# vitasoftAI/ImageRetrievalResearch

Hardware: AMD Instinct MI355X
Metric: images/sec embed + queries/sec top-k@100k-gallery, EffNet-B3a 224^2 (higher is better)
Workload: dtype bf16

## Files before the change

imageretrievalresearch_amd/csrc/gemm_bf16.hip:

```cpp
#include "ops.h"
#include "../../include/mi355_retrieval.h"

#include <stdlib.h>

namespace mi355 {

typedef __bf16 bf16x8 __attribute__((ext_vector_type(8)));
typedef float f32x4 __attribute__((ext_vector_type(4)));
typedef unsigned u32x4 __attribute__((ext_vector_type(4)));
typedef unsigned u32x2 __attribute__((ext_vector_type(2)));

__device__ __forceinline__ float lo_bf(unsigned u) { return __uint_as_float(u << 16); }
__device__ __forceinline__ float hi_bf(unsigned u) { return __uint_as_float(u & 0xffff0000u); }

__device__ __forceinline__ u32x4 gate_chunk(u32x4 v, const float* __restrict__ gp, int relu6) {
    const f32x4 g0 = *reinterpret_cast<const f32x4*>(gp);
    const f32x4 g1 = *reinterpret_cast<const f32x4*>(gp + 4);
    float f[8] = {lo_bf(v.x) * g0.x, hi_bf(v.x) * g0.y, lo_bf(v.y) * g0.z, hi_bf(v.y) * g0.w,
                  lo_bf(v.z) * g1.x, hi_bf(v.z) * g1.y, lo_bf(v.w) * g1.z, hi_bf(v.w) * g1.w};
    if (relu6) {
#pragma unroll
        for (int i = 0; i < 8; ++i) f[i] = fminf(fmaxf(f[i], 0.f), 6.f);
    }
    u32x4 o;
    o.x = pack2bf(f[0], f[1]); o.y = pack2bf(f[2], f[3]); o.z = pack2bf(f[4], f[5]); o.w = pack2bf(f[6], f[7]);
    return o;
}

__device__ __forceinline__ u32x4 gate_chunk_regs(u32x4 v, f32x4 g0, f32x4 g1, int relu6) {
    float f[8] = {lo_bf(v.x) * g0.x, hi_bf(v.x) * g0.y, lo_bf(v.y) * g0.z, hi_bf(v.y) * g0.w,
                  lo_bf(v.z) * g1.x, hi_bf(v.z) * g1.y, lo_bf(v.w) * g1.z, hi_bf(v.w) * g1.w};
    if (relu6) {
#pragma unroll
        for (int i = 0; i < 8; ++i) f[i] = fminf(fmaxf(f[i], 0.f), 6.f);
    }
    u32x4 o;
    o.x = pack2bf(f[0], f[1]); o.y = pack2bf(f[2], f[3]); o.z = pack2bf(f[4], f[5]); o.w = pack2bf(f[6], f[7]);
    return o;
}

__device__ __forceinline__ u32x4 relu6_chunk(u32x4 v) {
    float f[8] = {lo_bf(v.x), hi_bf(v.x), lo_bf(v.y), hi_bf(v.y), lo_bf(v.z), hi_bf(v.z), lo_bf(v.w), hi_bf(v.w)};
#pragma unroll
    for (int i = 0; i < 8; ++i) f[i] = fminf(fmaxf(f[i], 0.f), 6.f);
    u32x4 o;
    o.x = pack2bf(f[0], f[1]); o.y = pack2bf(f[2], f[3]); o.z = pack2bf(f[4], f[5]); o.w = pack2bf(f[6], f[7]);
    return o;
}

template <int WM, int NT, int BK>
__global__ __launch_bounds__(256) void k_gemm_bf16(const GemmArgs g, const int n_tiles, const int nwg) {
    constexpr int BM = 64 * WM;
    constexpr int BN = NT * 16;
    constexpr int LD = BK + 8;
    constexpr int KC = BK / 8;
    constexpr int A_ITERS = BM * KC / 256;
    constexpr int W_ITERS = (BN * KC + 255) / 256;
    constexpr int CLD = BN + 8;
    extern __shared__ __attribute__((aligned(16))) bf16_t smem[];
    bf16_t* As = smem;
    bf16_t* Ws = smem + 2 * BM * LD;

    const int tid = threadIdx.x;
    const int lane = tid & 63;
    const int wave = tid >> 6;

    int logical;
    {
        const int bid = blockIdx.x;
        const int q = nwg >> 3, r = nwg & 7, xcd = bid & 7;
        logical = (xcd < r ? xcd * (q + 1) : r * (q + 1) + (xcd - r) * q) + (bid >> 3);
    }
    const int mb = logical / n_tiles, nb = logical - mb * n_tiles;
    const int m0 = mb * BM;
    const int n0 = nb * BN;
    const int Npad = (g.N + 15) & ~15;

    const bf16_t* a_ptr[A_ITERS];
    const float* a_gate[A_ITERS];
    bool a_ok[A_ITERS];
    int a_lds[A_ITERS], a_k[A_ITERS];
#pragma unroll
    for (int i = 0; i < A_ITERS; ++i) {
        const int id = tid + 256 * i;
        const int row = id / KC, c = id % KC;
        const int m = m0 + row;
        a_ok[i] = m < g.M;
        a_k[i] = c * 8;
        a_lds[i] = row * LD + c * 8;
        a_ptr[i] = g.A + (size_t)(a_ok[i] ? m : 0) * g.lda + c * 8;
        a_gate[i] = g.gate ? g.gate + (size_t)((a_ok[i] ? m : 0) / g.rows_per_img) * g.gate_ld + c * 8 : nullptr;
    }

    u32x4 ra[A_ITERS], rw[W_ITERS];
    auto load_tile = [&](int k0) {
#pragma unroll
        for (int i = 0; i < A_ITERS; ++i) {
            u32x4 v = {0u, 0u, 0u, 0u};
            if (a_ok[i] && (k0 + a_k[i]) < g.K) {
                v = *reinterpret_cast<const u32x4*>(a_ptr[i] + k0);
                if (g.gate) v = gate_chunk(v, a_gate[i] + k0, g.a_relu6);
                else if (g.a_relu6) v = relu6_chunk(v);
            }
            ra[i] = v;
        }
#pragma unroll
        for (int i = 0; i < W_ITERS; ++i) {
            const int id = tid + 256 * i;
            const int row = id / KC, c = id % KC;
            u32x4 v = {0u, 0u, 0u, 0u};
            if (row < BN && (n0 + row) < Npad && (k0 + c * 8) < g.ldw)
                v = *reinterpret_cast<const u32x4*>(g.W + (size_t)(n0 + row) * g.ldw + k0 + c * 8);
            rw[i] = v;
        }
    };
    auto store_tile = [&](int buf) {
#pragma unroll
        for (int i = 0; i < A_ITERS; ++i) *reinterpret_cast<u32x4*>(&As[buf * BM * LD + a_lds[i]]) = ra[i];
#pragma unroll
        for (int i = 0; i < W_ITERS; ++i) {
            const int id = tid + 256 * i;
            const int row = id / KC, c = id % KC;
            if (row < BN) *reinterpret_cast<u32x4*>(&Ws[buf * BN * LD + row * LD + c * 8]) = rw[i];
        }
    };

    f32x4 acc[NT][WM];
#pragma unroll
    for (int i = 0; i < NT; ++i)
#pragma unroll
        for (int j = 0; j < WM; ++j) acc[i][j] = (f32x4){0.f, 0.f, 0.f, 0.f};

    const int nt = (g.K + BK - 1) / BK;
    load_tile(0);
    store_tile(0);
    __syncthreads();

    const int fr = lane & 15;
    const int fk = (lane >> 4) * 8;
    for (int t = 0; t < nt; ++t) {
        const int buf = t & 1;
        if (t + 1 < nt) load_tile((t + 1) * BK);
        const bf16_t* as = As + buf * BM * LD;
        const bf16_t* ws = Ws + buf * BN * LD;
#pragma unroll
        for (int ks = 0; ks < BK / 32; ++ks) {
            bf16x8 af[WM];
#pragma unroll
            for (int mi = 0; mi < WM; ++mi)
                af[mi] = *reinterpret_cast<const bf16x8*>(&as[(wave * 16 * WM + mi * 16 + fr) * LD + ks * 32 + fk]);
            constexpr int WG = NT % 4 == 0 ? 4 : (NT % 3 == 0 ? 3 : 2);
#pragma unroll
            for (int n0i = 0; n0i < NT; n0i += WG) {
                bf16x8 wf[WG];
#pragma unroll
                for (int q = 0; q < WG; ++q)
                    wf[q] = *reinterpret_cast<const bf16x8*>(&ws[((n0i + q) * 16 + fr) * LD + ks * 32 + fk]);
                __builtin_amdgcn_sched_barrier(0);
#pragma unroll
                for (int q = 0; q < WG; ++q)
#pragma unroll
                    for (int mi = 0; mi < WM; ++mi)
                        acc[n0i + q][mi] = __builtin_amdgcn_mfma_f32_16x16x32_bf16(wf[q], af[mi], acc[n0i + q][mi], 0, 0, 0);
            }
        }
        if (t + 1 < nt) store_tile(buf ^ 1);
        __syncthreads();
    }

    MI355_ACT_DISPATCH(g.act, {
_Pragma("unroll")
        for (int ni = 0; ni < NT; ++ni) {
            const int n = n0 + ni * 16 + (lane >> 4) * 4;
            f32x4 b = {0.f, 0.f, 0.f, 0.f};
            if (n < Npad) b = *reinterpret_cast<const f32x4*>(g.bias + n);
_Pragma("unroll")
            for (int mi = 0; mi < WM; ++mi) {
                acc[ni][mi].x = act_c<ACT>(acc[ni][mi].x + b.x); acc[ni][mi].y = act_c<ACT>(acc[ni][mi].y + b.y);
                acc[ni][mi].z = act_c<ACT>(acc[ni][mi].z + b.z); acc[ni][mi].w = act_c<ACT>(acc[ni][mi].w + b.w);
            }
        }
    })
    const bool staged = (!g.out_f32) && (g.res == nullptr);
    if (staged) {
        bf16_t* Cs = smem;
#pragma unroll
        for (int mi = 0; mi < WM; ++mi) {
            const int ml = wave * 16 * WM + mi * 16 + fr;
#pragma unroll
            for (int ni = 0; ni < NT; ++ni) {
                const int nl = ni * 16 + (lane >> 4) * 4;
                u32x2 o;
                o.x = pack2bf(acc[ni][mi].x, acc[ni][mi].y);
                o.y = pack2bf(acc[ni][mi].z, acc[ni][mi].w);
                *reinterpret_cast<u32x2*>(&Cs[ml * CLD + nl]) = o;
            }
        }
        __syncthreads();
        constexpr int CPR = BN / 8;
        for (int id = tid; id < BM * CPR; id += 256) {
            const int row = id / CPR, c = id - row * CPR;
            const int m = m0 + row, n = n0 + c * 8;
            if (m < g.M && n < g.N)
                *reinterpret_cast<u32x4*>((bf16_t*)g.out + (size_t)m * g.ldo + n) =
                    *reinterpret_cast<const u32x4*>(&Cs[row * CLD + c * 8]);
        }
        return;
    }
#pragma unroll
    for (int mi = 0; mi < WM; ++mi) {
        const int m = m0 + wave * 16 * WM + mi * 16 + fr;
        if (m >= g.M) continue;
#pragma unroll
        for (int ni = 0; ni < NT; ++ni) {
            const int n = n0 + ni * 16 + (lane >> 4) * 4;
            if (n >= g.N) continue;
            float v[4] = {acc[ni][mi].x, acc[ni][mi].y, acc[ni][mi].z, acc[ni][mi].w};
            const bool res_vec = g.res && (n + 3 < g.res_n);
            const bool res_part = g.res && !res_vec && (n < g.res_n);
            if (n + 3 < g.N && !res_part) {
                if (res_vec) {
                    const u32x2 rr = *reinterpret_cast<const u32x2*>(g.res + (size_t)m * g.ldr + n);
                    v[0] += lo_bf(rr.x); v[1] += hi_bf(rr.x); v[2] += lo_bf(rr.y); v[3] += hi_bf(rr.y);
                }
                if (g.out_f32) {
                    float* o = (float*)g.out + (size_t)m * g.ldo + n;
                    o[0] = v[0]; o[1] = v[1]; o[2] = v[2]; o[3] = v[3];
                } else {
                    u32x2 o;
                    o.x = pack2bf(v[0], v[1]);
                    o.y = pack2bf(v[2], v[3]);
                    *reinterpret_cast<u32x2*>((bf16_t*)g.out + (size_t)m * g.ldo + n) = o;
                }
            } else {
#pragma unroll
                for (int r = 0; r < 4; ++r) {
                    if (n + r < g.N) {
                        float x = v[r];
                        if (g.res && n + r < g.res_n) x += bf2f(g.res[(size_t)m * g.ldr + n + r]);
                        if (g.out_f32) ((float*)g.out)[(size_t)m * g.ldo + n + r] = x;
                        else ((bf16_t*)g.out)[(size_t)m * g.ldo + n + r] = f2bf(x);
                    }
                }
            }
        }
    }
}

constexpr int BG_BM = 128, BG_BN = 128, BG_BK = 64;

__device__ __forceinline__ void glds16(const bf16_t* gsrc, bf16_t* lds_dst) {
    __builtin_amdgcn_global_load_lds((const __attribute__((address_space(1))) void*)gsrc,
                                     (__attribute__((address_space(3))) void*)lds_dst, 16, 0, 0);
}

template <bool GATED, bool KTAIL, int BKT = 64>
__global__ __launch_bounds__(256, BKT == 32 ? 3 : 1) void k_gemm_big(const GemmArgs g, const int n_tiles, const int nwg) {
    constexpr int MI = GATED ? 2 : 4;
    constexpr int NI = GATED ? 8 : 4;
    static_assert(BKT == 64 || (BKT == 32 && !GATED), "stage depths");
    constexpr int PPW = BKT / 16;
    constexpr int RPP = 512 / BKT;
    constexpr int CPRW = BKT / 8;
    extern __shared__ __attribute__((aligned(16))) bf16_t bsm[];
    bf16_t* As = bsm;
    bf16_t* Ws = bsm + 2 * BG_BM * BKT;
    auto swz = [](int row) { return BKT == 64 ? ((row >> 1) & 7) : ((0 - (row >> 2)) & 3); };
    const int tid = threadIdx.x, lane = tid & 63, wave = tid >> 6;
    int logical;
    {
        const int bid = blockIdx.x;
        const int q = nwg >> 3, r = nwg & 7, xcd = bid & 7;
        logical = (xcd < r ? xcd * (q + 1) : r * (q + 1) + (xcd - r) * q) + (bid >> 3);
    }
    const int mb = logical / n_tiles, nb = logical - mb * n_tiles;
    const int m0 = mb * BG_BM, n0 = nb * BG_BN;
    const int Npad = (g.N + 15) & ~15;

    const bf16_t* a_src[PPW];
    const bf16_t* w_src[PPW];
    int k_off[PPW];
    bool a_ok[PPW], w_ok[PPW];
#pragma unroll
    for (int i = 0; i < PPW; ++i) {
        const int row = (wave * PPW + i) * RPP + lane / CPRW;
        const int lchunk = (lane % CPRW) ^ swz(row);
        k_off[i] = lchunk * 8;
        a_ok[i] = (m0 + row) < g.M;
        w_ok[i] = (n0 + row) < Npad;
        a_src[i] = g.A + (size_t)(a_ok[i] ? m0 + row : 0) * g.lda + lchunk * 8;
        w_src[i] = g.W + (size_t)(w_ok[i] ? n0 + row : 0) * g.ldw + lchunk * 8;
    }
    auto stage = [&](int buf, int k0) {
#pragma unroll
        for (int i = 0; i < PPW; ++i) {
            const int piece = wave * PPW + i;
            const bf16_t* pa = KTAIL ? ((a_ok[i] && k0 + k_off[i] < g.K) ? a_src[i] + k0 : g.zeros) : a_src[i] + k0;
            const bf16_t* pw = KTAIL ? ((w_ok[i] && k0 + k_off[i] < g.ldw) ? w_src[i] + k0 : g.zeros) : w_src[i] + k0;
            glds16(pa, As + buf * BG_BM * BKT + piece * 512);
            glds16(pw, Ws + buf * BG_BN * BKT + piece * 512);
        }
    };

    const int wm = GATED ? wave : (wave >> 1), wn = GATED ? 0 : (wave & 1);
    const int fr = lane & 15, fq = lane >> 4;
    const int row_base = wm * (MI * 16), col_base = wn * (NI * 16);
// ... 43 lines not shown
        const bf16_t* as = As + buf * BG_BM * BKT;
        const bf16_t* ws = Ws + buf * BG_BN * BKT;
#pragma unroll
        for (int ks = 0; ks < BKT / 32; ++ks) {
            bf16x8 af[MI], wf[NI];
#pragma unroll
            for (int i = 0; i < MI; ++i) {
                const int ra = row_base + i * 16 + fr;
                u32x4 v = *reinterpret_cast<const u32x4*>(&as[ra * BKT + (((ks * 4 + fq) ^ swz(ra)) << 3)]);
                if (GATED) {
                    if (g.gate) v = gate_chunk_regs(v, gcur[i][ks][0], gcur[i][ks][1], g.a_relu6);
                    else if (g.a_relu6) v = relu6_chunk(v);
                }
                af[i] = *reinterpret_cast<bf16x8*>(&v);
            }
#pragma unroll
            for (int i = 0; i < NI; ++i) {
                const int rw = col_base + i * 16 + fr;
                wf[i] = *reinterpret_cast<const bf16x8*>(&ws[rw * BKT + (((ks * 4 + fq) ^ swz(rw)) << 3)]);
            }
#pragma unroll
            for (int ni = 0; ni < NI; ++ni)
#pragma unroll
                for (int mi = 0; mi < MI; ++mi)
                    acc[ni][mi] = __builtin_amdgcn_mfma_f32_16x16x32_bf16(wf[ni], af[mi], acc[ni][mi], 0, 0, 0);
        }
        __syncthreads();
    }

    if (!GATED && g.ln_stats) {
        float mean[MI], rstd[MI];
#pragma unroll
        for (int mi = 0; mi < MI; ++mi) {
            const int m = min(m0 + row_base + mi * 16 + fr, g.M - 1);
            const mi355_f32x2 st = *reinterpret_cast<const mi355_f32x2*>(g.ln_stats + (size_t)m * 2);
            mean[mi] = st.x; rstd[mi] = st.y;
        }
#pragma unroll
        for (int ni = 0; ni < NI; ++ni) {
            const int n = n0 + col_base + ni * 16 + fq * 4;
            f32x4 cs = {0.f, 0.f, 0.f, 0.f};
            if (n < Npad) cs = *reinterpret_cast<const f32x4*>(g.ln_colsum + n);
#pragma unroll
            for (int mi = 0; mi < MI; ++mi) {
                acc[ni][mi].x = rstd[mi] * (acc[ni][mi].x - mean[mi] * cs.x); acc[ni][mi].y = rstd[mi] * (acc[ni][mi].y - mean[mi] * cs.y);
                acc[ni][mi].z = rstd[mi] * (acc[ni][mi].z - mean[mi] * cs.z); acc[ni][mi].w = rstd[mi] * (acc[ni][mi].w - mean[mi] * cs.w);
            }
        }
    }
    MI355_ACT_DISPATCH(g.act, {
_Pragma("unroll")
        for (int ni = 0; ni < NI; ++ni) {
            const int n = n0 + col_base + ni * 16 + fq * 4;
            f32x4 b = {0.f, 0.f, 0.f, 0.f};
            if (n < Npad) b = *reinterpret_cast<const f32x4*>(g.bias + n);
_Pragma("unroll")
            for (int mi = 0; mi < MI; ++mi) {
                acc[ni][mi].x = act_c<ACT>(acc[ni][mi].x + b.x); acc[ni][mi].y = act_c<ACT>(acc[ni][mi].y + b.y);
                acc[ni][mi].z = act_c<ACT>(acc[ni][mi].z + b.z); acc[ni][mi].w = act_c<ACT>(acc[ni][mi].w + b.w);
            }
        }
    })
    const bool staged = (!g.out_f32) && (g.res == nullptr);
    if (staged) {
        constexpr int CLD = BG_BN + 8;
        bf16_t* Cs = bsm;
#pragma unroll
        for (int mi = 0; mi < MI; ++mi) {
            const int ml = row_base + mi * 16 + fr;
#pragma unroll
            for (int ni = 0; ni < NI; ++ni) {
                const int nl = col_base + ni * 16 + fq * 4;
                u32x2 o;
                o.x = pack2bf(acc[ni][mi].x, acc[ni][mi].y);
                o.y = pack2bf(acc[ni][mi].z, acc[ni][mi].w);
                *reinterpret_cast<u32x2*>(&Cs[ml * CLD + nl]) = o;
            }
        }
        __syncthreads();
        constexpr int CPR = BG_BN / 8;
        for (int id = tid; id < BG_BM * CPR; id += 256) {
            const int row = id / CPR, c = id - row * CPR;
            const int m = m0 + row, n = n0 + c * 8;
            if (m < g.M && n < g.N)
                *reinterpret_cast<u32x4*>((bf16_t*)g.out + (size_t)m * g.ldo + n) =
                    *reinterpret_cast<const u32x4*>(&Cs[row * CLD + c * 8]);
        }
        return;
    }
    if (!g.out_f32 && g.res_n >= g.N) {
        constexpr int FLD = BG_BN + 4;
        float* Cf = reinterpret_cast<float*>(bsm);
        constexpr int HALVES = BKT == 32 ? 2 : 1, HROWS = BG_BM / HALVES;
#pragma unroll
        for (int h = 0; h < HALVES; ++h) {
            if (HALVES == 1 || row_base / HROWS == h) {
#pragma unroll
                for (int mi = 0; mi < MI; ++mi) {
                    const int ml = row_base + mi * 16 + fr - h * HROWS;
#pragma unroll
                    for (int ni = 0; ni < NI; ++ni) {
                        const int nl = col_base + ni * 16 + fq * 4;
                        *reinterpret_cast<f32x4*>(&Cf[ml * FLD + nl]) = acc[ni][mi];
                    }
                }
            }
            __syncthreads();
            constexpr int CPR = BG_BN / 8;
            for (int id = tid; id < HROWS * CPR; id += 256) {
                const int row = id / CPR, c = id - row * CPR;
                const int m = m0 + h * HROWS + row, n = n0 + c * 8;
                if (m < g.M && n < g.N) {
                    const f32x4 c0 = *reinterpret_cast<const f32x4*>(&Cf[row * FLD + c * 8]);
                    const f32x4 c1 = *reinterpret_cast<const f32x4*>(&Cf[row * FLD + c * 8 + 4]);
                    const u32x4 rr = *reinterpret_cast<const u32x4*>(g.res + (size_t)m * g.ldr + n);
                    u32x4 o;
                    o.x = pack2bf(c0.x + lo_bf(rr.x), c0.y + hi_bf(rr.x));
                    o.y = pack2bf(c0.z + lo_bf(rr.y), c0.w + hi_bf(rr.y));
                    o.z = pack2bf(c1.x + lo_bf(rr.z), c1.y + hi_bf(rr.z));
                    o.w = pack2bf(c1.z + lo_bf(rr.w), c1.w + hi_bf(rr.w));
                    *reinterpret_cast<u32x4*>((bf16_t*)g.out + (size_t)m * g.ldo + n) = o;
                }
            }
            if (h + 1 < HALVES) __syncthreads();
        }
        return;
    }
#pragma unroll
    for (int mi = 0; mi < MI; ++mi) {
        const int m = m0 + row_base + mi * 16 + fr;
        if (m >= g.M) continue;
#pragma unroll
        for (int ni = 0; ni < NI; ++ni) {
            const int n = n0 + col_base + ni * 16 + fq * 4;
            if (n >= g.N) continue;
            float v[4] = {acc[ni][mi].x, acc[ni][mi].y, acc[ni][mi].z, acc[ni][mi].w};
#pragma unroll
            for (int r = 0; r < 4; ++r) {
                if (n + r < g.N) {
                    float x = v[r];
                    if (g.res && n + r < g.res_n) x += bf2f(g.res[(size_t)m * g.ldr + n + r]);
                    v[r] = x;
                }
            }
            if (n + 3 < g.N && !g.out_f32) {
                u32x2 o;
                o.x = pack2bf(v[0], v[1]);
                o.y = pack2bf(v[2], v[3]);
                *reinterpret_cast<u32x2*>((bf16_t*)g.out + (size_t)m * g.ldo + n) = o;
            } else {
#pragma unroll
                for (int r = 0; r < 4; ++r) {
                    if (n + r < g.N) {
                        if (g.out_f32) ((float*)g.out)[(size_t)m * g.ldo + n + r] = v[r];
                        else ((bf16_t*)g.out)[(size_t)m * g.ldo + n + r] = f2bf(v[r]);
                    }
                }
            }
        }
    }
}

template <bool GATED, bool KTAIL, int BKT = 64>
static int launch_big(const GemmArgs& a, hipStream_t st) {
    const size_t lds = BKT == 64 ? (size_t)BG_BM * (BG_BN + 4) * 4 : (size_t)BG_BM * (BG_BN + 8) * 2;
    static bool attr_done[MI355_MAX_DEVICES] = {false};
    if (first_time_on_this_device(attr_done)) {
        MI355_CHECK_HIP(hipFuncSetAttribute((const void*)k_gemm_big<GATED, KTAIL, BKT>, hipFuncAttributeMaxDynamicSharedMemorySize,
                                            (int)lds));
    }
    const int n_tiles = cdiv(a.N, BG_BN), m_tiles = cdiv(a.M, BG_BM);
    const long nwg = (long)n_tiles * m_tiles;
    MI355_REQUIRE(nwg < (1l << 31), "gemm: grid too large");
    hipLaunchKernelGGL((k_gemm_big<GATED, KTAIL, BKT>), dim3((unsigned)nwg), dim3(256), lds, st, a, n_tiles, (int)nwg);
    MI355_LAUNCH_CHECK();
    return OK;
}

template <int NT, int KST>
__global__ __launch_bounds__(256) void k_gemm_stream(const GemmArgs g) {
    constexpr int PF = KST == 1 ? 4 : (KST <= 2 ? 3 : 1);
    constexpr int WLD = KST * 32 + 8;
    constexpr int CLD = NT * 16 + 8;
    extern __shared__ __attribute__((aligned(16))) bf16_t wsm[];
    const int tid = threadIdx.x, lane = tid & 63, wave = tid >> 6;
    const int Npad = (g.N + 15) & ~15;
    for (int id = tid; id < NT * 16 * KST * 4; id += 256) {
        const int row = id / (KST * 4), c = id - row * (KST * 4);
        u32x4 v = {0u, 0u, 0u, 0u};
        if (row < Npad && c * 8 < g.ldw) v = *reinterpret_cast<const u32x4*>(g.W + (size_t)row * g.ldw + c * 8);
        *reinterpret_cast<u32x4*>(&wsm[row * WLD + c * 8]) = v;
    }
    {
        float* sb = reinterpret_cast<float*>(wsm + NT * 16 * WLD + 4 * 16 * CLD);
        for (int n = tid; n < NT * 16; n += 256) sb[n] = n < Npad ? g.bias[n] : 0.f;
    }
    __syncthreads();

    bf16_t* cst = wsm + NT * 16 * WLD + wave * 16 * CLD;
    const float* sbias = reinterpret_cast<const float*>(wsm + NT * 16 * WLD + 4 * 16 * CLD);
    const int fr = lane & 15, fq = lane >> 4;
    const int nslabs = (g.M + 15) >> 4;
    const int stride = gridDim.x * 4;
    int slab = blockIdx.x * 4 + wave;

    auto load_slab = [&](int sl, u32x4 (&dst)[KST]) {
        const int m = sl * 16 + fr;
#pragma unroll
        for (int ks = 0; ks < KST; ++ks) {
            u32x4 v = {0u, 0u, 0u, 0u};
            const int k = ks * 32 + fq * 8;
            if (sl < nslabs && m < g.M && k < g.K) {
                v = *reinterpret_cast<const u32x4*>(g.A + (size_t)m * g.lda + k);
                if (g.gate) v = gate_chunk(v, g.gate + (size_t)(m / g.rows_per_img) * g.gate_ld + k, g.a_relu6);
                else if (g.a_relu6) v = relu6_chunk(v);
            }
            dst[ks] = v;
        }
    };

    u32x4 ring[PF][KST];
#pragma unroll
    for (int p = 0; p < PF; ++p) load_slab(slab + p * stride, ring[p]);


    while (slab < nslabs) {
#pragma unroll
        for (int p = 0; p < PF; ++p) {
            const int sl = slab + p * stride;
            if (sl < nslabs) {
                f32x4 acc[NT];
#pragma unroll
                for (int ni = 0; ni < NT; ++ni) acc[ni] = (f32x4){0.f, 0.f, 0.f, 0.f};
#pragma unroll
                for (int ks = 0; ks < KST; ++ks) {
                    const bf16x8 af = *reinterpret_cast<bf16x8*>(&ring[p][ks]);
#pragma unroll
                    for (int ni = 0; ni < NT; ++ni) {
                        const bf16x8 wf = *reinterpret_cast<const bf16x8*>(&wsm[(ni * 16 + fr) * WLD + ks * 32 + fq * 8]);
                        acc[ni] = __builtin_amdgcn_mfma_f32_16x16x32_bf16(wf, af, acc[ni], 0, 0, 0);
                    }
                }
                load_slab(sl + PF * stride, ring[p]);
                MI355_ACT_DISPATCH(g.act, {
_Pragma("unroll")
                    for (int ni = 0; ni < NT; ++ni) {
                        const f32x4 bb = *reinterpret_cast<const f32x4*>(&sbias[ni * 16 + fq * 4]);
                        acc[ni].x = act_c<ACT>(acc[ni].x + bb.x); acc[ni].y = act_c<ACT>(acc[ni].y + bb.y);
                        acc[ni].z = act_c<ACT>(acc[ni].z + bb.z); acc[ni].w = act_c<ACT>(acc[ni].w + bb.w);
                    }
                })
                const int m = sl * 16 + fr;
#pragma unroll
                for (int ni = 0; ni < NT; ++ni) {
                    const int n = ni * 16 + fq * 4;
                    float v[4] = {acc[ni].x, acc[ni].y, acc[ni].z, acc[ni].w};
                    if (g.res && m < g.M && n < g.N) {
                        if (n + 3 < g.res_n) {
                            const u32x2 rr = *reinterpret_cast<const u32x2*>(g.res + (size_t)m * g.ldr + n);
                            v[0] += lo_bf(rr.x); v[1] += hi_bf(rr.x); v[2] += lo_bf(rr.y); v[3] += hi_bf(rr.y);
                        } else {
#pragma unroll
                            for (int r = 0; r < 4; ++r)
                                if (n + r < g.res_n) v[r] += bf2f(g.res[(size_t)m * g.ldr + n + r]);
                        }
                    }
                    u32x2 o;
                    o.x = pack2bf(v[0], v[1]);
                    o.y = pack2bf(v[2], v[3]);
                    *reinterpret_cast<u32x2*>(&cst[fr * CLD + n]) = o;
                }
                constexpr int CPR = NT * 2;
#pragma unroll
                for (int i = 0; i < (16 * CPR + 63) / 64; ++i) {
                    const int id = lane + 64 * i;
                    const int row = id / CPR, c = id - row * CPR;
                    const int mm = sl * 16 + row;
                    if (id < 16 * CPR && mm < g.M && c * 8 < g.N)
                        *reinterpret_cast<u32x4*>((bf16_t*)g.out + (size_t)mm * g.ldo + c * 8) =
                            *reinterpret_cast<const u32x4*>(&cst[row * CLD + c * 8]);
                }
            }
        }
        slab += PF * stride;
    }
}

template <int NT, int KST>
static int launch_stream_cfg(const GemmArgs& a, hipStream_t st) {
    const size_t lds = (size_t)NT * 16 * (KST * 32 + 8) * 2 + (size_t)4 * 16 * (NT * 16 + 8) * 2 + (size_t)NT * 16 * 4;
    static bool attr_done[MI355_MAX_DEVICES] = {false};
    if (first_time_on_this_device(attr_done)) {
        MI355_CHECK_HIP(hipFuncSetAttribute((const void*)k_gemm_stream<NT, KST>,
                                            hipFuncAttributeMaxDynamicSharedMemorySize, 64 * 1024));
    }
    const int nslabs = cdiv(a.M, 16);
    int blocks = cdiv(nslabs, 4);
    if (blocks > 256 * 8) blocks = 256 * 8;
    hipLaunchKernelGGL((k_gemm_stream<NT, KST>), dim3(blocks), dim3(256), lds, st, a);
    MI355_LAUNCH_CHECK();
    return OK;
}

template <int NT, int KST>
__global__ __launch_bounds__(512) void k_proj_lds(const GemmArgs g) {
    constexpr int NW = 8;
    constexpr int KP = KST * 32;
    constexpr int WLD = KP + 8, ALD = KP + 8, CLD = NT * 16 + 8;
    extern __shared__ __attribute__((aligned(16))) unsigned char psm[];
    bf16_t* Wsh = reinterpret_cast<bf16_t*>(psm);
    float* sbias = reinterpret_cast<float*>(psm + (size_t)NT * 16 * WLD * 2);
    unsigned char* wbase = psm + (size_t)NT * 16 * WLD * 2 + NT * 16 * 4;
    constexpr int WS = 16 * ALD * 2 + 16 * CLD * 2 + KP * 4;
    const int tid = threadIdx.x, lane = tid & 63;
    const int wave = __builtin_amdgcn_readfirstlane(tid >> 6);
    bf16_t* As = reinterpret_cast<bf16_t*>(wbase + (size_t)wave * WS);
    bf16_t* Cs = As + 16 * ALD;
    float* Gs = reinterpret_cast<float*>(Cs + 16 * CLD);
    const int Npad = (g.N + 15) & ~15;
    for (int id = tid; id < NT * 16 * KST * 4; id += 512) {
        const int row = id / (KST * 4), c = id - row * (KST * 4);
        u32x4 v = {0u, 0u, 0u, 0u};
        if (row < Npad && c * 8 < g.ldw) v = *reinterpret_cast<const u32x4*>(g.W + (size_t)row * g.ldw + c * 8);
        *reinterpret_cast<u32x4*>(&Wsh[row * WLD + c * 8]) = v;
    }
    for (int n = tid; n < NT * 16; n += 512) sbias[n] = n < Npad ? g.bias[n] : 0.f;
    for (int id = lane; id < 16 * (ALD / 8); id += 64) *reinterpret_cast<u32x4*>(&As[id * 8]) = (u32x4){0u, 0u, 0u, 0u};
    __syncthreads();

    const int fr = lane & 15, fq = lane >> 4;
    const int kc = g.K >> 3;
    const int nchunk = 16 * kc;
    const int ntiles = (g.M + 15) >> 4;
    const int stride = gridDim.x * NW;
    int img = -1;
    u32x4 sv[KST];
    auto stage_load = [&](int tile) {
#pragma unroll
        for (int i = 0; i < KST; ++i) {
            const int id = min(lane + 64 * i, nchunk - 1);
            const int row = id / kc, c = id - row * kc;
            const int m = min(tile * 16 + row, g.M - 1);
            sv[i] = *reinterpret_cast<const u32x4*>(g.A + (size_t)m * g.lda + c * 8);
        }
        __builtin_amdgcn_sched_barrier(0);
    };
    int tile = blockIdx.x * NW + wave;
    if (tile < ntiles) stage_load(tile);
    for (; tile < ntiles; tile += stride) {
        if (g.gate) {
            const int im = (tile * 16) / g.rows_per_img;
            if (im != img) {
                img = im;
                for (int k4 = lane; k4 * 4 < g.K; k4 += 64)
                    *reinterpret_cast<f32x4*>(&Gs[k4 * 4]) = *reinterpret_cast<const f32x4*>(g.gate + (size_t)im * g.gate_ld + k4 * 4);
            }
        }
#pragma unroll
        for (int i = 0; i < KST; ++i) {
            const int id = lane + 64 * i;
            if (id < nchunk) {
                const int row = id / kc, c = id - row * kc;
                u32x4 v = sv[i];
                if (g.gate) v = gate_chunk(v, Gs + c * 8, g.a_relu6);
                else if (g.a_relu6) v = relu6_chunk(v);
                *reinterpret_cast<u32x4*>(&As[row * ALD + c * 8]) = v;
            }
        }
        if (tile + stride < ntiles) stage_load(tile + stride);
        f32x4 acc[NT];
#pragma unroll
        for (int ni = 0; ni < NT; ++ni) acc[ni] = (f32x4){0.f, 0.f, 0.f, 0.f};
#pragma unroll
        for (int ks = 0; ks < KST; ++ks) {
            const bf16x8 af = *reinterpret_cast<const bf16x8*>(&As[fr * ALD + ks * 32 + fq * 8]);
#pragma unroll
            for (int ni = 0; ni < NT; ++ni) {
                const bf16x8 wf = *reinterpret_cast<const bf16x8*>(&Wsh[(ni * 16 + fr) * WLD + ks * 32 + fq * 8]);
                acc[ni] = __builtin_amdgcn_mfma_f32_16x16x32_bf16(wf, af, acc[ni], 0, 0, 0);
            }
        }
        MI355_ACT_DISPATCH(g.act, {
_Pragma("unroll")
            for (int ni = 0; ni < NT; ++ni) {
                const f32x4 bb = *reinterpret_cast<const f32x4*>(&sbias[ni * 16 + fq * 4]);
                acc[ni].x = act_c<ACT>(acc[ni].x + bb.x); acc[ni].y = act_c<ACT>(acc[ni].y + bb.y);
                acc[ni].z = act_c<ACT>(acc[ni].z + bb.z); acc[ni].w = act_c<ACT>(acc[ni].w + bb.w);
            }
        })
        const int m = tile * 16 + fr;
#pragma unroll
        for (int ni = 0; ni < NT; ++ni) {
            const int n = ni * 16 + fq * 4;
            float v[4] = {acc[ni].x, acc[ni].y, acc[ni].z, acc[ni].w};
            if (g.res && m < g.M && n < g.N) {
                if (n + 3 < g.res_n) {
                    const u32x2 rr = *reinterpret_cast<const u32x2*>(g.res + (size_t)m * g.ldr + n);
                    v[0] += lo_bf(rr.x); v[1] += hi_bf(rr.x); v[2] += lo_bf(rr.y); v[3] += hi_bf(rr.y);
                } else {
#pragma unroll
                    for (int r = 0; r < 4; ++r)
                        if (n + r < g.res_n) v[r] += bf2f(g.res[(size_t)m * g.ldr + n + r]);
                }
            }
            u32x2 o;
            o.x = pack2bf(v[0], v[1]);
            o.y = pack2bf(v[2], v[3]);
            *reinterpret_cast<u32x2*>(&Cs[fr * CLD + n]) = o;
        }
        constexpr int CPR = NT * 2;
#pragma unroll
        for (int i = 0; i < (16 * CPR + 63) / 64; ++i) {
            const int id = lane + 64 * i;
            const int row = id / CPR, c = id - row * CPR;
            const int mm = tile * 16 + row;
            if (id < 16 * CPR && mm < g.M && c * 8 < g.N)
                *reinterpret_cast<u32x4*>((bf16_t*)g.out + (size_t)mm * g.ldo + c * 8) =
                    *reinterpret_cast<const u32x4*>(&Cs[row * CLD + c * 8]);
        }
    }
}

template <int NT, int KST>
static int launch_proj_cfg(const GemmArgs& a, hipStream_t st) {
    constexpr int KP = KST * 32;
    const size_t lds = (size_t)NT * 16 * (KP + 8) * 2 + (size_t)NT * 16 * 4 +
                       (size_t)8 * (16 * (KP + 8) * 2 + 16 * (NT * 16 + 8) * 2 + KP * 4);
    static bool attr_done[MI355_MAX_DEVICES] = {false};
    if (first_time_on_this_device(attr_done)) {
        MI355_CHECK_HIP(hipFuncSetAttribute((const void*)k_proj_lds<NT, KST>, hipFuncAttributeMaxDynamicSharedMemorySize,
                                            160 * 1024));
    }
    const int ntiles = cdiv(a.M, 16);
    int blocks = cdiv(ntiles, 8);
    if (blocks > 256 * 6) blocks = 256 * 6;
    hipLaunchKernelGGL((k_proj_lds<NT, KST>), dim3(blocks), dim3(512), lds, st, a);
    MI355_LAUNCH_CHECK();
    return OK;
}

static int try_launch_proj(const GemmArgs& a, hipStream_t st, int* nt_out) {
    if (a.out_f32 || a.M < (1 << 19) || a.N % 8 || a.ldo % 8 || a.N > 64 || a.K > 288 || a.lda != a.K) return -1;
    if (a.gate && (a.rows_per_img % 16 != 0 || a.gate_ld % 4 != 0)) return -1;
    const int kst = (a.K + 31) / 32, nt = (a.N + 15) / 16;
#define PROJ_CASE(NTV, KSTV) if (nt == NTV && kst == KSTV) { *nt_out = NTV; return launch_proj_cfg<NTV, KSTV>(a, st); }
    PROJ_CASE(2, 1); PROJ_CASE(2, 2); PROJ_CASE(2, 5); PROJ_CASE(2, 6); PROJ_CASE(3, 6); PROJ_CASE(3, 9); PROJ_CASE(2, 9);
    PROJ_CASE(4, 8); PROJ_CASE(3, 5);
#undef PROJ_CASE
    return -1;
}

static int try_launch_stream(const GemmArgs& a, hipStream_t st, int* nt_out) {
    if (a.out_f32 || a.M < 4096 || a.N % 8 || a.ldo % 8 || a.gate || a.a_relu6) return -1;
    const int kst = (a.K + 31) / 32;
    const int nt = (a.N + 15) / 16;
    *nt_out = nt;
    if (kst == 1 && nt == 9) return launch_stream_cfg<9, 1>(a, st);
    if (kst == 1 && nt == 12) return launch_stream_cfg<12, 1>(a, st);
    return -1;
}

constexpr int SK_KC = 256, SK_BM = 64, SK_BN = 64, SK_LD = SK_KC + 8;
constexpr size_t SK_MAX_BYTES = (size_t)64 << 20;

int gemm_splitk_chunks(long M, int rows_per_img, int N, int K) {
    if (M > 16384 || rows_per_img > 196 || K < 512 || N < 64 || N % 8 || gemm_splitk_bytes(M, N, K) > SK_MAX_BYTES) return 0;
    return (K + SK_KC - 1) / SK_KC;
}
size_t gemm_splitk_bytes(long M, int N, int K) {
    return (size_t)((K + SK_KC - 1) / SK_KC) * (size_t)M * (size_t)((N + 15) & ~15) * sizeof(float);
}

__global__ __launch_bounds__(256) void k_gemm_splitk(const GemmArgs g, float* __restrict__ ws) {
    extern __shared__ __attribute__((aligned(16))) bf16_t sksm[];
    bf16_t* As = sksm;
    bf16_t* Ws = sksm + SK_BM * SK_LD;
    const int tid = threadIdx.x, lane = tid & 63, wave = tid >> 6;
    const int n0 = blockIdx.x * SK_BN, m0 = blockIdx.y * SK_BM, k0 = blockIdx.z * SK_KC;
    const int Npad = (g.N + 15) & ~15;
    u32x4 ra[8], rw[8];
#pragma unroll
    for (int i = 0; i < 8; ++i) {
        const int id = tid + 256 * i;
        const int row = id >> 5, c = id & 31;
        const int k = k0 + c * 8;
        const int m = min(m0 + row, g.M - 1), kk = min(k, g.K - 8);
        ra[i] = *reinterpret_cast<const u32x4*>(g.A + (size_t)m * g.lda + kk);
        const int n = min(n0 + row, Npad - 1), kw = min(k, g.ldw - 8);
        rw[i] = *reinterpret_cast<const u32x4*>(g.W + (size_t)n * g.ldw + kw);
    }
#pragma unroll
    for (int i = 0; i < 8; ++i) {
        const int id = tid + 256 * i;
        const int row = id >> 5, c = id & 31;
        const int k = k0 + c * 8;
        u32x4 v = ra[i];
        if (m0 + row < g.M && k < g.K) {
            if (g.gate) v = gate_chunk(v, g.gate + (size_t)((m0 + row) / g.rows_per_img) * g.gate_ld + k, g.a_relu6);
            else if (g.a_relu6) v = relu6_chunk(v);
        } else {
            v = (u32x4){0u, 0u, 0u, 0u};
        }
        *reinterpret_cast<u32x4*>(&As[row * SK_LD + c * 8]) = v;
        u32x4 w = rw[i];
        if (n0 + row >= Npad || k >= g.ldw) w = (u32x4){0u, 0u, 0u, 0u};
        *reinterpret_cast<u32x4*>(&Ws[row * SK_LD + c * 8]) = w;
    }
    __syncthreads();
    const int fr = lane & 15, fq = lane >> 4;
    const int wm = wave >> 1, wn = wave & 1;
    f32x4 acc[2][2];
#pragma unroll
    for (int j = 0; j < 2; ++j)
#pragma unroll
        for (int i = 0; i < 2; ++i) acc[j][i] = (f32x4){0.f, 0.f, 0.f, 0.f};
#pragma unroll
    for (int ks = 0; ks < SK_KC / 32; ++ks) {
        bf16x8 af[2], wf[2];
#pragma unroll
        for (int i = 0; i < 2; ++i) af[i] = *reinterpret_cast<const bf16x8*>(&As[(wm * 32 + i * 16 + fr) * SK_LD + ks * 32 + fq * 8]);
#pragma unroll
        for (int j = 0; j < 2; ++j) wf[j] = *reinterpret_cast<const bf16x8*>(&Ws[(wn * 32 + j * 16 + fr) * SK_LD + ks * 32 + fq * 8]);
#pragma unroll
        for (int j = 0; j < 2; ++j)
#pragma unroll
            for (int i = 0; i < 2; ++i) acc[j][i] = __builtin_amdgcn_mfma_f32_16x16x32_bf16(wf[j], af[i], acc[j][i], 0, 0, 0);
    }
    float* wsk = ws + (size_t)blockIdx.z * g.M * Npad;
#pragma unroll
    for (int i = 0; i < 2; ++i) {
        const int m = m0 + wm * 32 + i * 16 + fr;
#pragma unroll
        for (int j = 0; j < 2; ++j) {
            const int n = n0 + wn * 32 + j * 16 + fq * 4;
            if (m < g.M && n < Npad) *reinterpret_cast<f32x4*>(wsk + (size_t)m * Npad + n) = acc[j][i];
        }
    }
}

__global__ __launch_bounds__(256) void k_splitk_reduce(const GemmArgs g, const float* __restrict__ ws, int nchunks) {
    const int Npad = (g.N + 15) & ~15, n4s = Npad >> 2;
    const long t = (long)blockIdx.x * 256 + threadIdx.x;
    if (t >= (long)g.M * n4s) return;
    const int m = (int)(t / n4s), n = (int)(t - (long)m * n4s) * 4;
    if (n >= g.N) return;
    f32x4 s = *reinterpret_cast<const f32x4*>(ws + (size_t)m * Npad + n);
    for (int c = 1; c < nchunks; ++c) {
        const f32x4 p = *reinterpret_cast<const f32x4*>(ws + ((size_t)c * g.M + m) * Npad + n);
        s.x += p.x; s.y += p.y; s.z += p.z; s.w += p.w;
    }
    const f32x4 bb = *reinterpret_cast<const f32x4*>(g.bias + n);
    float v[4] = {apply_act(s.x + bb.x, g.act), apply_act(s.y + bb.y, g.act), apply_act(s.z + bb.z, g.act), apply_act(s.w + bb.w, g.act)};
    if (g.res) {
#pragma unroll
        for (int r = 0; r < 4; ++r)
            if (n + r < g.res_n) v[r] += bf2f(g.res[(size_t)m * g.ldr + n + r]);
    }
    u32x2 o;
    o.x = pack2bf(v[0], v[1]);
    o.y = pack2bf(v[2], v[3]);
    *reinterpret_cast<u32x2*>((bf16_t*)g.out + (size_t)m * g.ldo + n) = o;
}

static int launch_splitk(const GemmArgs& a, int nchunks, hipStream_t st) {
    const size_t lds = (size_t)(SK_BM + SK_BN) * SK_LD * 2;
    static bool attr_done[MI355_MAX_DEVICES] = {false};
    if (first_time_on_this_device(attr_done)) {
        MI355_CHECK_HIP(hipFuncSetAttribute((const void*)k_gemm_splitk, hipFuncAttributeMaxDynamicSharedMemorySize, (int)lds));
    }
    const int Npad = (a.N + 15) & ~15;
    hipLaunchKernelGGL(k_gemm_splitk, dim3((unsigned)cdiv(Npad, SK_BN), (unsigned)cdiv(a.M, SK_BM), (unsigned)nchunks), dim3(256), lds, st,
                       a, a.splitk_ws);
    MI355_LAUNCH_CHECK();
    hipLaunchKernelGGL(k_splitk_reduce, dim3((unsigned)cdiv((long)a.M * (Npad / 4), 256)), dim3(256), 0, st, a,
                       (const float*)a.splitk_ws, nchunks);
    MI355_LAUNCH_CHECK();
    return OK;
}

static int pick_nt(int N, int max_nt = 12) {
    static const int opts[] = {2, 3, 4, 6, 8, 9, 12};
    int best = 2;
    double best_cost = 1e30;
    for (int nt : opts) {
        if (nt > max_nt) continue;
        const int bn = nt * 16;
        const int tiles = (N + bn - 1) / bn;
        const double cost = (double)tiles * bn * (1.0 + 24.0 / bn) + 8.0 * tiles;
        if (cost < best_cost) { best_cost = cost; best = nt; }
    }
    return best;
}

template <int WM, int NT, int BK>
static int launch_cfg(const GemmArgs& a, hipStream_t st) {
    constexpr int BM = 64 * WM, BN = NT * 16, LD = BK + 8;
    constexpr size_t stage = (size_t)2 * (BM + BN) * LD * 2, ctile = (size_t)BM * (BN + 8) * 2;
    constexpr size_t lds = stage > ctile ? stage : ctile;
    static bool attr_done[MI355_MAX_DEVICES] = {false};
    if (first_time_on_this_device(attr_done)) {
        MI355_CHECK_HIP(hipFuncSetAttribute((const void*)k_gemm_bf16<WM, NT, BK>,
                                            hipFuncAttributeMaxDynamicSharedMemorySize, (int)lds));
    }
    const int n_tiles = cdiv(a.N, BN);
    const int m_tiles = cdiv(a.M, BM);
    const long nwg = (long)n_tiles * m_tiles;
    MI355_REQUIRE(nwg < (1l << 31), "gemm: grid too large");
    hipLaunchKernelGGL((k_gemm_bf16<WM, NT, BK>), dim3((unsigned)nwg), dim3(256), lds, st, a, n_tiles, (int)nwg);
    MI355_LAUNCH_CHECK();
    return OK;
}

template <int WM, int BK>
static int launch_nt(const GemmArgs& a, int nt, hipStream_t st) {
    switch (nt) {
        case 2: return launch_cfg<WM, 2, BK>(a, st);
        case 3: return launch_cfg<WM, 3, BK>(a, st);
        case 4: return launch_cfg<WM, 4, BK>(a, st);
        case 6: return launch_cfg<WM, 6, BK>(a, st);
        case 8: return launch_cfg<WM, 8, BK>(a, st);
        case 9: return launch_cfg<WM, 9, BK>(a, st);
        default: return launch_cfg<WM, 12, BK>(a, st);
    }
}

constexpr int HG_NT = 128;
constexpr int HG_SLD = HG_NT + 8;

static int head_gap_wld(int K) { return ((K + 31) & ~31) + 8; }
static size_t head_gap_lds_bytes(int K) {
    return (size_t)HG_NT * head_gap_wld(K) * sizeof(bf16_t) + (size_t)4 * 16 * HG_SLD * sizeof(bf16_t);
}

template <int ACT, int KSMAX>
__global__ __launch_bounds__(256) void k_head_gap(const bf16_t* __restrict__ A, int lda, const bf16_t* __restrict__ W, int ldw,
                                                  const float* __restrict__ bias, float* __restrict__ pooled,
                                                  bf16_t* __restrict__ pooled_bf16, int ldp, int B, int HW, int N, int K) {
    extern __shared__ __attribute__((aligned(16))) bf16_t hg_sm[];
    const int tid = threadIdx.x, lane = tid & 63, wave = tid >> 6;
    const int fr = lane & 15, fq = lane >> 4;
    const int n0 = blockIdx.x * HG_NT;
    const int Npad = (N + 15) & ~15;
    const int nks = (K + 31) >> 5;
    const int WLD = nks * 32 + 8;
    bf16_t* Ws = hg_sm;
    bf16_t* strip = hg_sm + HG_NT * WLD + wave * 16 * HG_SLD;
    {
        const int cpr = nks * 4;
        for (int i = tid; i < HG_NT * cpr; i += 256) {
            const int r = i / cpr, c = i - r * cpr;
            *reinterpret_cast<u32x4*>(&Ws[r * WLD + c * 8]) =
                *reinterpret_cast<const u32x4*>(W + (size_t)min(n0 + r, Npad - 1) * ldw + c * 8);
        }
    }
    __syncthreads();
    const int b = blockIdx.y * 4 + wave;
    if (b >= B) return;
    const bf16_t* Ab = A + (size_t)b * HW * lda;
    const bf16_t* arow[4];
#pragma unroll
    for (int mi = 0; mi < 4; ++mi) arow[mi] = Ab + (size_t)min(mi * 16 + fr, HW - 1) * lda;
    f32x4 acc[8][4];
#pragma unroll
    for (int ni = 0; ni < 8; ++ni)
#pragma unroll
        for (int mi = 0; mi < 4; ++mi) acc[ni][mi] = (f32x4){0.f, 0.f, 0.f, 0.f};
    u32x4 af[3][4];
    auto load = [&](int s, int ks) {
        const int ka = min(ks * 32 + fq * 8, lda - 8);
#pragma unroll
        for (int mi = 0; mi < 4; ++mi) af[s][mi] = *reinterpret_cast<const u32x4*>(arow[mi] + ka);
    };
    load(0, 0);
    if (nks > 1) load(1, 1);
#pragma unroll
    for (int ks = 0; ks < KSMAX; ++ks) {
        if (ks < nks) {
            if (ks + 2 < nks) load((ks + 2) % 3, ks + 2);
#pragma unroll
            for (int ni = 0; ni < 8; ++ni) {
                const u32x4 wf = *reinterpret_cast<const u32x4*>(&Ws[(ni * 16 + fr) * WLD + ks * 32 + fq * 8]);
#pragma unroll
                for (int mi = 0; mi < 4; ++mi)
                    acc[ni][mi] = __builtin_amdgcn_mfma_f32_16x16x32_bf16(*reinterpret_cast<const bf16x8*>(&wf),
                                                                          *reinterpret_cast<const bf16x8*>(&af[ks % 3][mi]),
                                                                          acc[ni][mi], 0, 0, 0);
            }
        }
    }
    f32x4 bb[8];
#pragma unroll
    for (int ni = 0; ni < 8; ++ni) {
        const int n = n0 + ni * 16 + fq * 4;
        bb[ni] = n < Npad ? *reinterpret_cast<const f32x4*>(bias + n) : (f32x4){0.f, 0.f, 0.f, 0.f};
    }
    float s0 = 0.f, s1 = 0.f;
#pragma unroll
    for (int mi = 0; mi < 4; ++mi) {
        if (mi * 16 >= HW) break;
#pragma unroll
        for (int ni = 0; ni < 8; ++ni) {
            const f32x4 a = acc[ni][mi];
            u32x2 o;
            o.x = pack2bf(act_c<ACT>(a.x + bb[ni].x), act_c<ACT>(a.y + bb[ni].y));
            o.y = pack2bf(act_c<ACT>(a.z + bb[ni].z), act_c<ACT>(a.w + bb[ni].w));
            *reinterpret_cast<u32x2*>(&strip[fr * HG_SLD + ni * 16 + fq * 4]) = o;
        }
        const int np = min(16, HW - mi * 16);
        for (int i = 0; i < np; ++i) {
            const unsigned v = *reinterpret_cast<const unsigned*>(&strip[i * HG_SLD + 2 * lane]);
            s0 += __uint_as_float(v << 16);
            s1 += __uint_as_float(v & 0xffff0000u);
        }
    }
    const int n = n0 + 2 * lane;
    if (n < N) {
        s0 *= 1.0f / (float)HW;
        s1 *= 1.0f / (float)HW;
        *reinterpret_cast<float2*>(&pooled[(size_t)b * ldp + n]) = make_float2(s0, s1);
        if (pooled_bf16) {
            pooled_bf16[(size_t)b * ldp + n] = f2bf(s0);
            pooled_bf16[(size_t)b * ldp + n + 1] = f2bf(s1);
        }
    }
}

bool head_gap_supported(int HW, int N, int K, int lda, int ldw, int act) {
    return HW >= 1 && HW <= 64 && K >= 32 && K <= 512 && lda % 8 == 0 && lda >= 8 && ldw % 32 == 0 && ldw >= ((K + 31) & ~31) && N % 8 == 0 &&
           (act == ACT_SILU || act == ACT_NONE);
}

template <int ACT, int KSMAX>
static int launch_head_gap_cfg(const bf16_t* A, int lda, const bf16_t* W, int ldw, const float* bias, float* pooled,
                               bf16_t* pooled_bf16, int ldp, int B, int HW, int N, int K, hipStream_t st) {
    static bool attr_done[MI355_MAX_DEVICES] = {};
    if (first_time_on_this_device(attr_done))
        MI355_CHECK_HIP(hipFuncSetAttribute((const void*)k_head_gap<ACT, KSMAX>, hipFuncAttributeMaxDynamicSharedMemorySize,
                                            (int)head_gap_lds_bytes(KSMAX * 32)));
    const dim3 grid((unsigned)cdiv(N, HG_NT), (unsigned)cdiv(B, 4));
    hipLaunchKernelGGL((k_head_gap<ACT, KSMAX>), grid, dim3(256), head_gap_lds_bytes(K), st, A, lda, W, ldw, bias, pooled,
                       pooled_bf16, ldp, B, HW, N, K);
    MI355_LAUNCH_CHECK();
    return OK;
}

int launch_head_gap(const bf16_t* A, int lda, const bf16_t* W, int ldw, const float* bias, float* pooled, bf16_t* pooled_bf16,
// ... 78 lines not shown
```

Measured before the change: 61990.

## Prefetch gate and residual tiles, use contiguous tile ranges and occupancy-sized grid

The projection GEMM kernel now gives each block a contiguous range of tiles instead of a grid-strided interleave. Gate vectors and, for small K, residual rows are prefetched into registers one iteration ahead and staged through LDS, so their global latency overlaps the MFMA work. The grid size comes from an occupancy query rather than a fixed cap, and launch bounds request more waves per SIMD. The cost is higher register pressure from the prefetch buffers, plus per-launch hipGetDevice calls.

```diff
diff --git a/imageretrievalresearch_amd/csrc/gemm_bf16.hip b/imageretrievalresearch_amd/csrc/gemm_bf16.hip
--- a/imageretrievalresearch_amd/csrc/gemm_bf16.hip
+++ b/imageretrievalresearch_amd/csrc/gemm_bf16.hip
@@ -2,6 +2,9 @@
 #include "../../include/mi355_retrieval.h"
 
 #include <stdlib.h>
+
+#include <algorithm>
+#include <type_traits>
 
 namespace mi355 {
 
@@ -651,10 +654,25 @@
     return OK;
 }
 
+constexpr size_t proj_lds_bytes(int NT, int KST) {
+    return (size_t)NT * 16 * (KST * 32 + 8) * 2 + (size_t)NT * 16 * 4 +
+           (size_t)8 * (16 * (KST * 32 + 8) * 2 + 16 * (NT * 16 + 8) * 2 + KST * 32 * 4);
+}
+constexpr int proj_waves_per_simd(int NT, int KST) {
+    const int fit = (int)(160 * 1024 / proj_lds_bytes(NT, KST));
+    const int cap = KST == 1 ? 4 : 3;
+    return 2 * (fit > cap ? cap : fit < 1 ? 1 : fit);
+}
+
 template <int NT, int KST>
-__global__ __launch_bounds__(512) void k_proj_lds(const GemmArgs g) {
+__global__ __launch_bounds__(512, proj_waves_per_simd(NT, KST)) void k_proj_lds(const GemmArgs g) {
     constexpr int NW = 8;
+    constexpr bool RPF = KST <= 2;
     constexpr int KP = KST * 32;
+    constexpr int GW = KP <= 64 ? 1 : 4;
+    constexpr int GCH = (KP / GW + 63) / 64;
+    using gvec = typename std::conditional<GW == 1, float, f32x4>::type;
+    constexpr int RCH = (16 * NT * 2 + 63) / 64;
     constexpr int WLD = KP + 8, ALD = KP + 8, CLD = NT * 16 + 8;
     extern __shared__ __attribute__((aligned(16))) unsigned char psm[];
     bf16_t* Wsh = reinterpret_cast<bf16_t*>(psm);
@@ -681,28 +699,60 @@
     const int kc = g.K >> 3;
     const int nchunk = 16 * kc;
     const int ntiles = (g.M + 15) >> 4;
-    const int stride = gridDim.x * NW;
-    int img = -1;
+    const int per = ntiles / (int)gridDim.x, extra = ntiles - per * (int)gridDim.x;
+    const int t0 = (int)blockIdx.x * per + min((int)blockIdx.x, extra);
+    const int tend = t0 + per + ((int)blockIdx.x < extra ? 1 : 0);
+    const bool res_pf = RPF && g.res && g.res_n > 0 && g.res_n <= g.N && (g.res_n & 7) == 0 && (g.ldr & 7) == 0 &&
+                        ((size_t)g.res & 15) == 0;
+    const int rc = res_pf ? g.res_n >> 3 : 0;
+    int roff[RCH], rlds[RCH];
+#pragma unroll
+    for (int i = 0; i < RCH; ++i) {
+        const int rcs = max(rc, 1);
+        const int id = min(lane + 64 * i, 16 * rcs - 1);
+        const int row = id / rcs, c = id - row * rcs;
+        roff[i] = row * g.ldr + c * 8;
+        rlds[i] = row * CLD + c * 8;
+    }
+    int img_req = -1;
     u32x4 sv[KST];
-    auto stage_load = [&](int tile) {
-#pragma unroll
-        for (int i = 0; i < KST; ++i) {
-            const int id = min(lane + 64 * i, nchunk - 1);
-            const int row = id / kc, c = id - row * kc;
-            const int m = min(tile * 16 + row, g.M - 1);
-            sv[i] = *reinterpret_cast<const u32x4*>(g.A + (size_t)m * g.lda + c * 8);
+    u32x4 rv[RCH];
+    gvec gv[GCH];
+    bool gnew = false;
+    auto stage_load = [&](int t) {
+        if (g.gate) {
+            const int im = (t * 16) / g.rows_per_img;
+            gnew = im != img_req;
+            if (gnew) {
+                img_req = im;
+#pragma unroll
+                for (int i = 0; i < GCH; ++i) {
+                    const int k = (lane + 64 * i) * GW;
+                    if (k < g.K) gv[i] = *reinterpret_cast<const gvec*>(g.gate + (size_t)im * g.gate_ld + k);
+                }
+            }
+        }
+        const bf16_t* ab = g.A + (size_t)t * nchunk * 8;
+        const int alim = (g.M - t * 16) * kc - 1;
+#pragma unroll
+        for (int i = 0; i < KST; ++i)
+            sv[i] = *reinterpret_cast<const u32x4*>(ab + min(min(lane + 64 * i, nchunk - 1), alim) * 8);
+        if (rc) {
+            const bf16_t* rb = g.res + (size_t)t * 16 * g.ldr;
+            const int rlim = min(g.M - 1 - t * 16, 15) * g.ldr + (rc - 1) * 8;
+#pragma unroll
+            for (int i = 0; i < RCH; ++i) rv[i] = *reinterpret_cast<const u32x4*>(rb + min(roff[i], rlim));
         }
         __builtin_amdgcn_sched_barrier(0);
     };
-    int tile = blockIdx.x * NW + wave;
-    if (tile < ntiles) stage_load(tile);
-    for (; tile < ntiles; tile += stride) {
-        if (g.gate) {
-            const int im = (tile * 16) / g.rows_per_img;
-            if (im != img) {
-                img = im;
-                for (int k4 = lane; k4 * 4 < g.K; k4 += 64)
-                    *reinterpret_cast<f32x4*>(&Gs[k4 * 4]) = *reinterpret_cast<const f32x4*>(g.gate + (size_t)im * g.gate_ld + k4 * 4);
+    int tile = t0 + wave;
+    if (tile < tend) stage_load(tile);
+    for (; tile < tend; tile += NW) {
+        if (g.gate && gnew) {
+#pragma unroll
+            for (int i = 0; i < GCH; ++i) {
+                const int k = (lane + 64 * i) * GW;
+                if (k < g.K) *reinterpret_cast<gvec*>(&Gs[k]) = gv[i];
             }
         }
 #pragma unroll
@@ -716,7 +766,12 @@
                 *reinterpret_cast<u32x4*>(&As[row * ALD + c * 8]) = v;
             }
         }
-        if (tile + stride < ntiles) stage_load(tile + stride);
+        if (rc) {
+#pragma unroll
+            for (int i = 0; i < RCH; ++i)
+                if (lane + 64 * i < 16 * rc) *reinterpret_cast<u32x4*>(&Cs[rlds[i]]) = rv[i];
+        }
+        if (tile + NW < tend) stage_load(tile + NW);
         f32x4 acc[NT];
 #pragma unroll
         for (int ni = 0; ni < NT; ++ni) acc[ni] = (f32x4){0.f, 0.f, 0.f, 0.f};
@@ -742,7 +797,12 @@
         for (int ni = 0; ni < NT; ++ni) {
             const int n = ni * 16 + fq * 4;
             float v[4] = {acc[ni].x, acc[ni].y, acc[ni].z, acc[ni].w};
-            if (g.res && m < g.M && n < g.N) {
+            if (rc) {
+                if (n < g.res_n) {
+                    const u32x2 rr = *reinterpret_cast<const u32x2*>(&Cs[fr * CLD + n]);
+                    v[0] += lo_bf(rr.x); v[1] += hi_bf(rr.x); v[2] += lo_bf(rr.y); v[3] += hi_bf(rr.y);
+                }
+            } else if (g.res && m < g.M && n < g.N) {
                 if (n + 3 < g.res_n) {
                     const u32x2 rr = *reinterpret_cast<const u32x2*>(g.res + (size_t)m * g.ldr + n);
                     v[0] += lo_bf(rr.x); v[1] += hi_bf(rr.x); v[2] += lo_bf(rr.y); v[3] += hi_bf(rr.y);
@@ -762,9 +822,8 @@
         for (int i = 0; i < (16 * CPR + 63) / 64; ++i) {
             const int id = lane + 64 * i;
             const int row = id / CPR, c = id - row * CPR;
-            const int mm = tile * 16 + row;
-            if (id < 16 * CPR && mm < g.M && c * 8 < g.N)
-                *reinterpret_cast<u32x4*>((bf16_t*)g.out + (size_t)mm * g.ldo + c * 8) =
+            if (id < 16 * CPR && row < g.M - tile * 16 && c * 8 < g.N)
+                *reinterpret_cast<u32x4*>((bf16_t*)g.out + (size_t)tile * 16 * g.ldo + (row * g.ldo + c * 8)) =
                     *reinterpret_cast<const u32x4*>(&Cs[row * CLD + c * 8]);
         }
     }
@@ -772,17 +831,21 @@
 
 template <int NT, int KST>
 static int launch_proj_cfg(const GemmArgs& a, hipStream_t st) {
-    constexpr int KP = KST * 32;
-    const size_t lds = (size_t)NT * 16 * (KP + 8) * 2 + (size_t)NT * 16 * 4 +
-                       (size_t)8 * (16 * (KP + 8) * 2 + 16 * (NT * 16 + 8) * 2 + KP * 4);
-    static bool attr_done[MI355_MAX_DEVICES] = {false};
-    if (first_time_on_this_device(attr_done)) {
-        MI355_CHECK_HIP(hipFuncSetAttribute((const void*)k_proj_lds<NT, KST>, hipFuncAttributeMaxDynamicSharedMemorySize,
-                                            160 * 1024));
+    constexpr size_t lds = proj_lds_bytes(NT, KST);
+    static int slots[MI355_MAX_DEVICES] = {0};
+    int dev = 0;
+    MI355_CHECK_HIP(hipGetDevice(&dev));
+    MI355_REQUIRE(dev >= 0 && dev < MI355_MAX_DEVICES, "gemm: device ordinal %d out of range", dev);
+    if (!slots[dev]) {
+        const void* fn = (const void*)k_proj_lds<NT, KST>;
+        MI355_CHECK_HIP(hipFuncSetAttribute(fn, hipFuncAttributeMaxDynamicSharedMemorySize, 160 * 1024));
+        int per_cu = 0, cus = 0;
+        MI355_CHECK_HIP(hipOccupancyMaxActiveBlocksPerMultiprocessor(&per_cu, fn, 512, lds));
+        MI355_CHECK_HIP(hipDeviceGetAttribute(&cus, hipDeviceAttributeMultiprocessorCount, dev));
+        slots[dev] = (per_cu > 0 ? per_cu : 1) * (cus > 0 ? cus : 256);
     }
     const int ntiles = cdiv(a.M, 16);
-    int blocks = cdiv(ntiles, 8);
-    if (blocks > 256 * 6) blocks = 256 * 6;
+    const int blocks = std::min(slots[dev], cdiv(ntiles, 8));
     hipLaunchKernelGGL((k_proj_lds<NT, KST>), dim3(blocks), dim3(512), lds, st, a);
     MI355_LAUNCH_CHECK();
     return OK;
@@ -791,6 +854,7 @@
 static int try_launch_proj(const GemmArgs& a, hipStream_t st, int* nt_out) {
     if (a.out_f32 || a.M < (1 << 19) || a.N % 8 || a.ldo % 8 || a.N > 64 || a.K > 288 || a.lda != a.K) return -1;
     if (a.gate && (a.rows_per_img % 16 != 0 || a.gate_ld % 4 != 0)) return -1;
+    if ((long)a.M * a.K >= (1L << 34)) return -1;
     const int kst = (a.K + 31) / 32, nt = (a.N + 15) / 16;
 #define PROJ_CASE(NTV, KSTV) if (nt == NTV && kst == KSTV) { *nt_out = NTV; return launch_proj_cfg<NTV, KSTV>(a, st); }
     PROJ_CASE(2, 1); PROJ_CASE(2, 2); PROJ_CASE(2, 5); PROJ_CASE(2, 6); PROJ_CASE(3, 6); PROJ_CASE(3, 9); PROJ_CASE(2, 9);
```

New measurement: 62410, median of 6. No clear change (+0.7%).
